# Samirez/Visual_odometry

Hardware: AMD Instinct MI355X
Metric: frame-pairs/sec (1280x720, 2000 ORB feats) (higher is better)
Workload: dtype u8+f32+f64; 1 GPU; seeded synthetic 1280x720 drone flight (256 distinct rendered views, closed loop), 2000 ORB features/frame, 8 levels = BASELINE config 2; chunk of 257 consecutive frames -> 256 pairs (k, k+1) per GPU per step, each frame detected once; detector=orb, distinct_rendered_frames=256, pair_stride=1, contexts_per_gpu=3, keypoint_order=cv2, poly_solver=fast, matcher=crosscheck, matcher_kernel=mfma_fp4, ransac=5-point, conf 0.99, 1 px, seed 2^64-1, <=1000 iters, parallelism=single GPU, pairs_ok_last_step=256

## Files before the change

### visual_odometry_amd/csrc/orb_kernels.hip

```cpp
#include "vo_internal.h"
#include <type_traits>
#include <float.h>
#include <stdlib.h>

__constant__ int8_t c_pattern[256 * 4] = {
#include "orb_pattern.inc"
};
__constant__ int c_umax[16] = {15, 15, 15, 15, 14, 14, 14, 13, 13, 12, 11, 10, 9, 8, 6, 3};
__constant__ int c_gauss7[7] = {18, 34, 49, 55, 49, 34, 18};


typedef short vo_s16x2 __attribute__((ext_vector_type(2)));
typedef unsigned short vo_u16x2 __attribute__((ext_vector_type(2)));
__device__ __forceinline__ uint32_t pk_sub16(uint32_t a, uint32_t b)
{
    return __builtin_bit_cast(uint32_t, __builtin_bit_cast(vo_s16x2, a) - __builtin_bit_cast(vo_s16x2, b));
}
__device__ __forceinline__ uint32_t pk_add16(uint32_t a, uint32_t b)
{
    return __builtin_bit_cast(uint32_t, __builtin_bit_cast(vo_s16x2, a) + __builtin_bit_cast(vo_s16x2, b));
}
__device__ __forceinline__ uint32_t pk_min16(uint32_t a, uint32_t b)
{
    return __builtin_bit_cast(uint32_t, __builtin_elementwise_min(__builtin_bit_cast(vo_s16x2, a), __builtin_bit_cast(vo_s16x2, b)));
}
__device__ __forceinline__ uint32_t pk_max16(uint32_t a, uint32_t b)
{
    return __builtin_bit_cast(uint32_t, __builtin_elementwise_max(__builtin_bit_cast(vo_s16x2, a), __builtin_bit_cast(vo_s16x2, b)));
}
__device__ __forceinline__ uint32_t pk_lshr16_8(uint32_t a)
{
    return __builtin_bit_cast(uint32_t, __builtin_bit_cast(vo_u16x2, a) >> (unsigned short)8);
}
__device__ __forceinline__ uint32_t swap16(uint32_t a) { return __builtin_amdgcn_alignbit(a, a, 16); }

__device__ __forceinline__ int wave_incl_scan(int v, int lane)
{
#pragma unroll
    for (int d = 1; d < 64; d <<= 1) {
        int t = __shfl_up(v, d, 64);
        if (lane >= d) v += t;
    }
    return v;
}

__device__ __forceinline__ int block_excl_scan(int v, int* s_w, int* total)
{
    const int tid = threadIdx.x, lane = tid & 63, wid = tid >> 6, nw = (blockDim.x + 63) >> 6;
    int inc = wave_incl_scan(v, lane);
    __syncthreads();
    if (lane == 63) s_w[wid] = inc;
    __syncthreads();
    if (wid == 0) {
        int w = lane < nw ? s_w[lane] : 0;
        int winc = wave_incl_scan(w, lane);
        if (lane < nw) s_w[lane] = winc - w;
        if (lane == nw - 1) s_w[16] = winc;
    }
// ... 1045 lines not shown
    const LevelGeom lv = g.lv[l];
    const int n = min(ff.cand_count[f * VO_MAX_LEVELS + l], lv.cand_cap);
    const uint32_t* pos = ff.cand_pos + (size_t)f * g.cand_total + lv.cand_off;
    const float* resp = ff.cand_resp + (size_t)f * g.cand_total + lv.cand_off;
    const float thr = thr_in[f * VO_MAX_LEVELS + l];
    int out_base = 0;
    for (int k = 0; k < l; k++) out_base += kept_in[f * VO_MAX_LEVELS + k];
    uint32_t* kp_pos = ff.kp_pos + (size_t)f * g.kp_cap;
    int* kp_level = ff.kp_level + (size_t)f * g.kp_cap;
    float* kp_resp = ff.kp_resp + (size_t)f * g.kp_cap;
    bool overflow = false;
    for (int base = 0; base < n; base += 256) {
        const int i = base + tid;
        const bool keep = i < n && resp[i] >= thr;
        int tot;
        const int p = out_base + block_excl_scan(keep ? 1 : 0, s_w, &tot);
        if (keep) {
            if (p < g.kp_cap) { kp_pos[p] = pos[i]; kp_level[p] = l; kp_resp[p] = resp[i]; }
            else overflow = true;
        }
        out_base += tot;
    }
    if (overflow) atomicOr(&ff.flags[f], 1);
    if (l == g.nlevels - 1 && tid == 0) ff.kp_count[f] = min(out_base, g.kp_cap);
}

void launch_select_harris(hipStream_t s, const PyrGeom& g, FrameFeat ff, int F, float* thr, int* kept)
{
    hipLaunchKernelGGL(k_harris_threshold, dim3(g.nlevels, F), dim3(256), 0, s, g, ff, thr, kept);
    hipLaunchKernelGGL(k_harris_compact, dim3(g.nlevels, F), dim3(256), 0, s, g, ff, thr, kept);
}

__device__ __forceinline__ float fast_atan2_deg(float y, float x)
{
    const float p1 = 0.9997878412794807f * (float)(180 / 3.1415926535897932384626433832795);
    const float p3 = -0.3258083974640975f * (float)(180 / 3.1415926535897932384626433832795);
    const float p5 = 0.1555786518463281f * (float)(180 / 3.1415926535897932384626433832795);
    const float p7 = -0.04432655554792128f * (float)(180 / 3.1415926535897932384626433832795);
    float ax = fabsf(x), ay = fabsf(y), a, c, c2;
    if (ax >= ay) {
        c = ay / (ax + (float)DBL_EPSILON);
        c2 = c * c;
        a = (((p7 * c2 + p5) * c2 + p3) * c2 + p1) * c;
    } else {
        c = ax / (ay + (float)DBL_EPSILON);
        c2 = c * c;
        a = 90.f - (((p7 * c2 + p5) * c2 + p3) * c2 + p1) * c;
    }
    if (x < 0) a = 180.f - a;
    if (y < 0) a = 360.f - a;
    return a;
}

__constant__ uint32_t c_disc_mask[16][8] = {
#define DM(u0, um) ((((u0) >= -(um) && (u0) <= (um)) ? 0x000000ffu : 0u) | (((u0) + 1 >= -(um) && (u0) + 1 <= (um)) ? 0x0000ff00u : 0u) | \
                    (((u0) + 2 >= -(um) && (u0) + 2 <= (um)) ? 0x00ff0000u : 0u) | (((u0) + 3 >= -(um) && (u0) + 3 <= (um)) ? 0xff000000u : 0u))
#define DROW(um) {DM(-15, um), DM(-11, um), DM(-7, um), DM(-3, um), DM(1, um), DM(5, um), DM(9, um), DM(13, um)}
    DROW(15), DROW(15), DROW(15), DROW(15), DROW(14), DROW(14), DROW(14), DROW(13),
    DROW(13), DROW(12), DROW(11), DROW(10), DROW(9), DROW(8), DROW(6), DROW(3)
#undef DROW
#undef DM
};

#ifndef ANG_KPW
#define ANG_KPW 4
#endif
__global__ __launch_bounds__(256) void k_angle(const uint8_t* pyr, PyrGeom g, FrameFeat ff, int blocks_per_frame)
{
    const int bid = xcd_tile(blockIdx.x, gridDim.x);
    const int f = bid / blocks_per_frame, lane = threadIdx.x & 63;
    const int k0 = ((bid % blocks_per_frame) * 4 + (threadIdx.x >> 6)) * ANG_KPW;
    const int cnt = min(ff.kp_count[f], g.kp_cap);
    if (k0 >= cnt) return;
    const uint8_t* corner[ANG_KPW];
    int stride[ANG_KPW];
#pragma unroll
    for (int q = 0; q < ANG_KPW; q++) {
        const size_t ki = (size_t)f * g.kp_cap + min(k0 + q, cnt - 1);
        const uint32_t pos = __builtin_amdgcn_readfirstlane(ff.kp_pos[ki]);
        const int level = __builtin_amdgcn_readfirstlane(ff.kp_level[ki]);
        stride[q] = g.lv[level].stride;
        corner[q] = pyr + (size_t)f * g.frame_bytes + g.lv[level].off + (size_t)((int)(pos >> 16) - 15) * stride[q] + ((int)(pos & 0xffff) - 15);
    }
    uint32_t w[ANG_KPW][4];
#pragma unroll
    for (int q = 0; q < ANG_KPW; q++)
#pragma unroll
        for (int it = 0; it < 4; it++) {
            const int idx = min(it * 64 + lane, 247);
            __builtin_memcpy(&w[q][it], corner[q] + (size_t)(idx >> 3) * stride[q] + 4 * (idx & 7), 4);
        }
    float m10f = 0.f, m01f = 0.f;
#pragma unroll
    for (int q = 0; q < ANG_KPW; q++) {
        int m10 = 0, m01 = 0;
#pragma unroll
        for (int it = 0; it < 4; it++) {
            const int idx = it * 64 + lane;
            const int r = min(idx, 247) >> 3, j = idx & 7, v = r - 15, av = v < 0 ? -v : v;
            const uint32_t x = idx < 248 ? w[q][it] & c_disc_mask[av][j] : 0u;
            const int sum = (int)__builtin_amdgcn_udot4(x, 0x01010101u, 0u, false);
            const int wsum = (int)__builtin_amdgcn_udot4(x, 0x03020100u, 0u, false);
            m10 += (4 * j - 15) * sum + wsum;
            m01 += v * sum;
        }
#pragma unroll
        for (int d = 32; d >= 1; d >>= 1) { m10 += __shfl_xor(m10, d, 64); m01 += __shfl_xor(m01, d, 64); }
        if (lane == q) { m10f = (float)m10; m01f = (float)m01; }
    }
    if (lane < ANG_KPW && k0 + lane < cnt) ff.kp_angle[(size_t)f * g.kp_cap + k0 + lane] = fast_atan2_deg(m01f, m10f);
}

void launch_angle(hipStream_t s, const uint8_t* pyr, const PyrGeom& g, FrameFeat ff, int F)
{
    const int bpf = (g.kp_cap + 4 * ANG_KPW - 1) / (4 * ANG_KPW);
    hipLaunchKernelGGL(k_angle, dim3(bpf * F), dim3(256), 0, s, pyr, g, ff, bpf);
}

__device__ __forceinline__ int reflect101(int i, int n)
{
    if (n == 1) return 0;
    while (i < 0 || i >= n) i = i < 0 ? -i : 2 * n - 2 - i;
    return i;
}

#define BL_INW 160
#define BL_INH (BLUR_TH + 6)
#define BL_ROWS_PER_LANE (BLUR_TH / 8)

__global__ __launch_bounds__(256) void k_blur(const uint8_t* pyr, uint8_t* blur, PyrGeom g)
{
    __shared__ __attribute__((aligned(16))) uint8_t s_in[BL_INH * BL_INW];
    __shared__ __attribute__((aligned(16))) uint16_t s_h[BL_INH * BLUR_TW];
    const int f = blockIdx.y, tid = threadIdx.x;
    const int bid = xcd_tile(blockIdx.x, g.btiles_total);
    int l = 0;
    while (l + 1 < g.nlevels && bid >= g.lv[l + 1].btile_base) l++;
    const LevelGeom lv = g.lv[l];
    const int tile = bid - lv.btile_base;
    const int x0 = (tile % lv.btiles_x) * BLUR_TW, y0 = (tile / lv.btiles_x) * BLUR_TH;
    const uint8_t* img = pyr + (size_t)f * g.frame_bytes + lv.off;
    if (lv.w >= 16 && lv.h >= 4) {
        {
            constexpr int NCH = BL_INW / 16, RPS = 256 / NCH, NLD = (BL_INH + RPS - 1) / RPS;
            const int cc = tid % NCH, rr = tid / NCH;
            const bool lane_ok = tid < RPS * NCH;
            const int gx = x0 - 16 + 16 * cc;
            const bool inx = gx >= 0 && gx + 16 <= lv.stride;
            const uint8_t* src = img + min(max(gx, 0), lv.stride - 16);
            const bool rows_inside = y0 >= 3 && y0 + BLUR_TH + 3 <= lv.h;
            uint4 bv[NLD];
#pragma unroll
            for (int k = 0; k < NLD; k++) {
                const int ry = min(rr + RPS * k, BL_INH - 1);
                const int gy = rows_inside ? y0 - 3 + ry : reflect101(y0 - 3 + ry, lv.h);
                const uint4 v = *(const uint4*)(src + (size_t)gy * lv.stride);
                bv[k] = inx ? v : make_uint4(0, 0, 0, 0);
            }
#pragma unroll
            for (int k = 0; k < NLD; k++)
                if (lane_ok && rr + RPS * k < BL_INH) *(uint4*)(s_in + (rr + RPS * k) * BL_INW + 16 * cc) = bv[k];
        }
        const bool left = x0 == 0, right = x0 + BLUR_TW + 3 > lv.w;
        if (left || right) {
            __syncthreads();
            for (int i = tid; i < BL_INH * 6; i += 256) {
                const int ry = i / 6, k = i % 6;
                if (k < 3) {
                    if (left) s_in[ry * BL_INW + 16 - 3 + k] = s_in[ry * BL_INW + 16 + 3 - k];
                } else if (right) {
                    const int x = lv.w + (k - 3), sx = 2 * lv.w - 2 - x;
// ... 174 lines not shown
    const LevelGeom lv = g.lv[l];
    const int ntx = (lv.stride + 255) / 256, tile = wt - first;
    const int x0 = (tile % ntx) * 256, y0 = (tile / ntx) * BD_R;
    const int x = x0 + 4 * lane;
    const uint8_t* img = pyr + (size_t)f * g.frame_bytes + lv.off;
    const int xb = min(max(x - 4, 0), lv.stride - 12);
    BdEdge e;
    e.left = x0 == 0; e.right = x0 + 256 + 8 > lv.w;
    e.shl = x == 0; e.shr = x - 4 > lv.stride - 12 && x < lv.stride;
    {
        const int d = lv.w - x;
        e.s1 = d == 1 ? 0x01020304u : d == 2 ? 0x03040504u : d == 3 ? 0x05060504u : 0x07060504u;
        e.s2 = d == 2 ? 0x0c0c0c02u : d == 3 ? 0x0c0c0304u : 0x0c040506u;
        e.s3 = d == 5 ? 0x01020304u : d == 6 ? 0x03040504u : 0x07060504u;
        e.use_t = d >= 2 && d <= 4;
    }
    const __amdgpu_buffer_rsrc_t drs = __builtin_amdgcn_make_buffer_rsrc(blur + (size_t)f * g.frame_bytes + lv.off, 0, lv.stride * lv.h, 0x00020000);
    const bool col_ok = x < lv.stride;
    const int nout = min(BD_R, lv.h - y0);
    const int nsteps = (nout + 1) / 2;
    const bool inside = y0 >= 3 && y0 - 3 + 2 * (nsteps + 3 + BD_AHEAD) <= lv.h, edge = e.left || e.right;
    if (inside && !edge) bd_strip<true, false>(img, lv, drs, x, xb, y0, nout, nsteps, col_ok, e);
    else if (inside) bd_strip<true, true>(img, lv, drs, x, xb, y0, nout, nsteps, col_ok, e);
    else if (!edge) bd_strip<false, false>(img, lv, drs, x, xb, y0, nout, nsteps, col_ok, e);
    else bd_strip<false, true>(img, lv, drs, x, xb, y0, nout, nsteps, col_ok, e);
}

void launch_blur(hipStream_t s, const uint8_t* pyr, uint8_t* blur, const PyrGeom& g, int F)
{
    bool direct = true;
    int total = 0;
    for (int l = 0; l < g.nlevels; l++) {
        direct = direct && g.lv[l].w >= 16 && g.lv[l].h >= 8;
        total += ((g.lv[l].stride + 255) / 256) * ((g.lv[l].h + BD_R - 1) / BD_R);
    }
    if (direct) { hipLaunchKernelGGL(k_blur_direct, dim3((total + 3) / 4, F), dim3(256), 0, s, pyr, blur, g, total); return; }
    hipLaunchKernelGGL(k_blur, dim3(g.btiles_total, F), dim3(256), 0, s, pyr, blur, g);
}

__device__ __forceinline__ uint32_t brief_expand4(uint32_t nib)
{
    const uint32_t m = (nib * 0x00204081u) & 0x01010101u;
    return 0x81818181u ^ (m * 0xfeu);
}

__device__ __forceinline__ uint32_t brief_expand8_fp4(uint32_t b)
{
    uint32_t w = (b | (b << 12)) & 0x000F000Fu;
    w = (w | (w << 6)) & 0x03030303u;
    w = (w | (w << 3)) & 0x11111111u;
    return 0xAAAAAAAAu ^ (w << 3);
}

__global__ __launch_bounds__(256) void k_brief_trig(PyrGeom g, FrameFeat ff)
{
    const int f = blockIdx.y, k = blockIdx.x * 256 + threadIdx.x;
    if (k >= min(ff.kp_count[f], g.kp_cap)) return;
    const size_t ki = (size_t)f * g.kp_cap + k;
    const float angle = ff.kp_angle[ki] * (float)(3.1415926535897932384626433832795 / 180.f);
    ff.kp_xy[ki * 2] = (float)cos((double)angle);
    ff.kp_xy[ki * 2 + 1] = (float)sin((double)angle);
}

#define BR_R 18
#define BR_ROWS (2 * BR_R + 1)
#ifndef BR_KPW
#define BR_KPW 2
#endif
__global__ __launch_bounds__(256) void k_brief(const uint8_t* blur, PyrGeom g, FrameFeat ff, uint8_t* desc_x, int cap_x, int blocks_per_frame, int fp4)
{
    __shared__ __attribute__((aligned(16))) uint8_t s_win[4][BR_KPW][BR_ROWS * 64];
    const int bid = xcd_tile(blockIdx.x, gridDim.x);
    const int f = bid / blocks_per_frame, lane = threadIdx.x & 63, wave = threadIdx.x >> 6;
    const int k0 = ((bid % blocks_per_frame) * 4 + wave) * BR_KPW;
    const int cnt = min(ff.kp_count[f], g.kp_cap);
    if (k0 >= cnt) return;
    float ca[BR_KPW], cb[BR_KPW], kxs[BR_KPW], kys[BR_KPW], sfs[BR_KPW];
    int coff[BR_KPW];
    uint4 wv[BR_KPW][3];
#pragma unroll
    for (int q = 0; q < BR_KPW; q++) {
        const size_t ki = (size_t)f * g.kp_cap + min(k0 + q, cnt - 1);
        const uint32_t pos = __builtin_amdgcn_readfirstlane(ff.kp_pos[ki]);
        const int level = __builtin_amdgcn_readfirstlane(ff.kp_level[ki]);
        const float sf = g.lv[level].scale;
        const int stride = g.lv[level].stride, lh = g.lv[level].h;
        const float kx = (float)(pos & 0xffff) * sf, ky = (float)(pos >> 16) * sf;
        const float inv = 1.f / sf;
        const int cx = __float2int_rn(kx * inv), cy = __float2int_rn(ky * inv);
        ca[q] = ff.kp_xy[ki * 2]; cb[q] = ff.kp_xy[ki * 2 + 1];
        kxs[q] = kx; kys[q] = ky; sfs[q] = sf;
        const uint8_t* img = blur + (size_t)f * g.frame_bytes + g.lv[level].off;
        const int xs = (cx - BR_R) & ~15;
        const int nchunk = (cx - BR_R - xs) + 2 * BR_R + 1 > 48 ? 4 : 3;
        coff[q] = BR_R * 64 + (cx - xs);
#pragma unroll
        for (int it = 0; it < 3; it++) {
            const int idx = min(it * 64 + lane, BR_ROWS * 4 - 1);
            const int r = idx >> 2, c = idx & 3;
            const int gy = min(max(cy - BR_R + r, 0), lh - 1), gx = min(max(xs + (c < nchunk ? 16 * c : 0), 0), stride - 16);
            wv[q][it] = *(const uint4*)(img + (size_t)gy * stride + gx);
        }
    }
#pragma unroll
    for (int q = 0; q < BR_KPW; q++)
#pragma unroll
        for (int it = 0; it < 3; it++) {
            const int idx = it * 64 + lane;
            if (idx < BR_ROWS * 4) *(uint4*)(s_win[wave][q] + idx * 16) = wv[q][it];
        }
#pragma unroll
    for (int q = 0; q < BR_KPW; q++) {
        const int k = k0 + q;
        if (k >= cnt) break;
        const size_t ki = (size_t)f * g.kp_cap + k;
        const uint8_t* center = s_win[wave][q] + coff[q];
        const float a = ca[q], b = cb[q];
        uint64_t words[4];
#pragma unroll
        for (int w = 0; w < 4; w++) {
            const int8_t* pt = c_pattern + (w * 64 + lane) * 4;
            const float px0 = (float)pt[0], py0 = (float)pt[1], px1 = (float)pt[2], py1 = (float)pt[3];
            const float xa = px0 * a - py0 * b, ya = px0 * b + py0 * a;
            const float xb = px1 * a - py1 * b, yb = px1 * b + py1 * a;
            const int t0 = center[__float2int_rn(ya) * 64 + __float2int_rn(xa)];
            const int t1 = center[__float2int_rn(yb) * 64 + __float2int_rn(xb)];
            words[w] = __ballot(t0 < t1);
        }
        if (lane < 4) {
            uint64_t wv8 = lane == 0 ? words[0] : lane == 1 ? words[1] : lane == 2 ? words[2] : words[3];
            *(uint64_t*)(ff.desc + ki * 32 + lane * 8) = wv8;
        }
        if (fp4 < 0) {
        } else if (fp4) {
            if (lane < 8) {
                const uint64_t wv8 = lane < 2 ? words[0] : lane < 4 ? words[1] : lane < 6 ? words[2] : words[3];
                const uint32_t bits = (uint32_t)(wv8 >> (32 * (lane & 1)));
                const uint4 o = make_uint4(brief_expand8_fp4(bits & 255u), brief_expand8_fp4((bits >> 8) & 255u), brief_expand8_fp4((bits >> 16) & 255u), brief_expand8_fp4(bits >> 24));
                *(uint4*)(desc_x + ((size_t)f * cap_x * 16 + (size_t)(k & ~15) * 8 + (size_t)lane * 16 + (k & 15)) * 16) = o;
            }
        } else if (lane < 16) {
            const uint64_t wv8 = lane < 4 ? words[0] : lane < 8 ? words[1] : lane < 12 ? words[2] : words[3];
            const uint32_t bits = (uint32_t)(wv8 >> (16 * (lane & 3))) & 0xffffu;
            const uint4 o = make_uint4(brief_expand4(bits & 15u), brief_expand4((bits >> 4) & 15u), brief_expand4((bits >> 8) & 15u), brief_expand4(bits >> 12));
            *(uint4*)(desc_x + (((size_t)f * cap_x + (k & ~15)) * 16 + (size_t)lane * 16 + (k & 15)) * 16) = o;
        }
        if (lane == 0) {
            ff.kp_xy[ki * 2] = kxs[q]; ff.kp_xy[ki * 2 + 1] = kys[q];
            ff.kp_size[ki] = 31 * sfs[q];
        }
    }
}

void launch_brief(hipStream_t s, const uint8_t* blur, const PyrGeom& g, FrameFeat ff, int F, uint8_t* desc_x, int cap_x, int fp4)
{
    hipLaunchKernelGGL(k_brief_trig, dim3((g.kp_cap + 255) / 256, F), dim3(256), 0, s, g, ff);
    const int bpf = (g.kp_cap + 4 * BR_KPW - 1) / (4 * BR_KPW);
    hipLaunchKernelGGL(k_brief, dim3(bpf * F), dim3(256), 0, s, blur, g, ff, desc_x, cap_x, bpf, -1);
    launch_desc_expand(s, ff.desc, ff.kp_count, g.kp_cap, cap_x, desc_x, F, fp4);
}
```

### visual_odometry_amd/csrc/vo_api.hip

```cpp
#include "vo_host.h"

static const char* k_stage_names[VO_STAGE_COUNT] = {
    "gray", "pyramid_resize", "fast_score_nms", "select_fast", "harris", "select_harris", "ic_angle",
    "gaussian_blur", "rbrief", "match_nn", "match_select", "essential_ransac", "recover_pose",
    "triangulate", "misc", "reserved", "sift_scale_space", "sift_extrema", "sift_refine_orient", "sift_sort_unique",
    "sift_descriptor", "cv2_keypoint_order", "trajectory_gather", "reserved2", "slam_ba_prepare", "slam_bundle_adjust", "slam_filter",
    "slam_camera_limit", "slam_map_statistics", "undistort_points"};

static void clear_last_run(vo_ctx* ctx) { ctx->last = LastRun(); }

static void slam_stream_slots_written(vo_ctx* ctx, int first, int n)
{
    for (int k = first < 0 ? 0 : first; k < first + n && k < (int)ctx->undistorted.size(); k++) ctx->undistorted[(size_t)k] = 0;
    SlamStream& st = ctx->stream_map;
    if (st.live && st.anchor >= first && st.anchor < first + n) st.touched = true;
    for (SlamStream::Seq& q : st.seq)
        if (st.live && q.anchor >= first && q.anchor < first + n) q.touched = true;
}

void prof_collect(vo_ctx* c)
{
    for (int i = 0; i < c->n_ev; i++) {
        float ms = 0;
        if (hipEventElapsedTime(&ms, c->ev[i][0], c->ev[i][1]) == hipSuccess) {
// ... 449 lines not shown
    HIPCHK(hipStreamSynchronize(ctx->stream));
    if (ctx->prof) prof_collect(ctx);
    return VO_OK;
}

static int run_detect(vo_ctx* ctx, int first_slot, int F, int upto)
{
    const PyrGeom& g = ctx->g;
    hipStream_t s = ctx->stream;
    uint8_t* pyr = ctx->pyr + (size_t)first_slot * g.frame_bytes;
    uint8_t* blur = ctx->blur + (size_t)first_slot * g.frame_bytes;
    uint8_t* score = ctx->score + (size_t)first_slot * g.frame_bytes;
    FrameFeat ff = ctx->ff;
    ff.cand_pos += (size_t)first_slot * g.cand_total; ff.cand_resp += (size_t)first_slot * g.cand_total;
    ff.cand_count += (size_t)first_slot * VO_MAX_LEVELS;
    ff.kp_pos += (size_t)first_slot * g.kp_cap; ff.kp_level += (size_t)first_slot * g.kp_cap;
    ff.kp_resp += (size_t)first_slot * g.kp_cap; ff.kp_angle += (size_t)first_slot * g.kp_cap;
    ff.kp_xy += (size_t)first_slot * g.kp_cap * 2; ff.kp_size += (size_t)first_slot * g.kp_cap;
    ff.desc += (size_t)first_slot * g.kp_cap * 32;
    ff.kp_count += first_slot; ff.flags += first_slot;
    ff.hist += (size_t)first_slot * VO_MAX_LEVELS * 256;
    ff.tile_list += (size_t)first_slot * g.ftiles_total * FAST_LISTCAP; ff.tile_count += (size_t)first_slot * g.ftiles_total;
    {
        StageTimer t(ctx, ST_RESIZE);
        for (int l = 1; l < g.nlevels; l++) launch_resize(s, pyr, g, l, ctx->tabs[l], F);
    }
    if (upto < 1) return VO_OK;
    const bool cv2 = ctx->kp_order == 1 && ctx->cv2_ready;
    Cv2Buf cb = ctx->cv2;
    if (cv2) {
        const size_t fo = (size_t)first_slot;
        cb.all_pos += fo * cb.all_total; cb.all_resp += fo * cb.all_total; cb.work += fo * cb.all_total;
        cb.all_cand += fo * cb.all_total; cb.lpos += fo * cb.all_total; cb.rpos += fo * cb.all_total;
        cb.all_count += fo * VO_MAX_LEVELS; cb.chunk_count += fo * g.sel_chunks_total;
    }
    {
        StageTimer t(ctx, ST_MISC);
        HIPCHK(hipMemsetAsync(ff.hist, 0, (size_t)F * VO_MAX_LEVELS * 256 * sizeof(uint32_t), s));
        if (upto < 2) {
            HIPCHK(hipMemsetAsync(ff.flags, 0, (size_t)F * sizeof(int), s));
            HIPCHK(hipMemsetAsync(ff.cand_count, 0, (size_t)F * VO_MAX_LEVELS * sizeof(int), s));
            if (cv2) HIPCHK(hipMemsetAsync(cb.all_count, 0, (size_t)F * VO_MAX_LEVELS * sizeof(int), s));
        }
    }
    { StageTimer t(ctx, ST_FAST); launch_fast(s, pyr, score, ff.hist, g, F, upto < 2 ? nullptr : ff.tile_list, ff.tile_count); }
    if (upto < 2) return VO_OK;
    { StageTimer t(ctx, ST_SELECT_FAST); launch_select_fast(s, g, ff, F, ctx->sel_thr + (size_t)first_slot * VO_MAX_LEVELS, ctx->sel_chunk_count + (size_t)first_slot * g.sel_chunks_total, ff.tile_list, ff.tile_count, cv2 ? &cb : nullptr); }
    if (g.score_type == 0) { StageTimer t(ctx, ST_HARRIS); launch_harris(s, pyr, g, ff, F); }
    { StageTimer t(ctx, ST_SELECT_HARRIS); launch_select_harris(s, g, ff, F, ctx->har_thr + (size_t)first_slot * VO_MAX_LEVELS, ctx->har_kept + (size_t)first_slot * VO_MAX_LEVELS); }
    if (cv2) {
        StageTimer t(ctx, ST_CV2_ORDER);
        launch_cv2_order(s, g, ff, cb, F, ctx->har_kept + (size_t)first_slot * VO_MAX_LEVELS);
    }
    { StageTimer t(ctx, ST_ANGLE); launch_angle(s, pyr, g, ff, F); }
    { StageTimer t(ctx, ST_BLUR); launch_blur(s, pyr, blur, g, F); }
    {
        StageTimer t(ctx, ST_BRIEF);
        const int cx = desc_x_rows(g.kp_cap);
        const int fp4 = descx_begin_write(ctx, first_slot, F);
        launch_brief(s, blur, g, ff, F, ctx->desc_x + (size_t)first_slot * cx * 256, cx, fp4);
    }
    return VO_OK;
}

extern "C" int vo_batch_kp_capacity(vo_ctx* ctx)
{
    if (!ctx) return 0;
    const Batch b = batch(ctx);
    return b.ready ? b.kp_cap : 0;
}

extern "C" int vo_host_alloc(size_t bytes, void** out)
{
    if (!out) return VO_ERR_INVALID;
    *out = nullptr;
    return hipHostMalloc(out, bytes ? bytes : 1, hipHostMallocDefault) == hipSuccess ? VO_OK : VO_ERR_HIP;
}

extern "C" void vo_host_free(void* p)
{
    if (p) (void)hipHostFree(p);
}

static int detect_enqueue(vo_ctx* ctx, int first_slot, int F)
{
    const Batch b = batch(ctx);
    if (!b.ready) FAIL(VO_ERR_NOT_CONFIGURED, "vo_batch_configure has not been called");
    if (F < 0 || first_slot < 0 || first_slot + F > b.max_frames) FAIL(VO_ERR_INVALID, "slot range out of bounds");
    slam_stream_slots_written(ctx, first_slot, F);
    HIPCHK(hipSetDevice(ctx->device));
    if (F == 0) return VO_OK;
    if (b.sift) return sift_frames_detect_enqueue(ctx, first_slot, F);
    int rc = run_detect(ctx, first_slot, F, 2);
    if (rc) return rc;
    HIPCHK(hipGetLastError());
    return VO_OK;
}

extern "C" int vo_frames_detect_async(vo_ctx* ctx, int first_slot, int F)
{
    if (!ctx) return VO_ERR_INVALID;
    int rc = detect_enqueue(ctx, first_slot, F);
    if (rc) return rc;
    HIPCHK(hipEventRecord(ctx->ev_det, ctx->stream));
    ctx->ev_det_set = true;
    return VO_OK;
}

extern "C" int vo_detect_after(vo_ctx* ctx, vo_ctx* other)
{
    if (!ctx || !other) return VO_ERR_INVALID;
    if (ctx->device != other->device) FAIL(VO_ERR_INVALID, "the two contexts are on different devices");
    if (ctx == other || !other->ev_det_set) return VO_OK;
// ... 2019 lines not shown
    ctx->n_ev = 0;
    return VO_OK;
}

extern "C" int vo_profile_reset(vo_ctx* ctx)
{
    if (!ctx) return VO_ERR_INVALID;
    memset(ctx->prof_ms, 0, sizeof(ctx->prof_ms));
    memset(ctx->prof_n, 0, sizeof(ctx->prof_n));
    ctx->n_ev = 0;
    return VO_OK;
}

extern "C" int vo_profile_read(vo_ctx* ctx, float* ms, int32_t* launches)
{
    if (!ctx || !ms || !launches) return VO_ERR_INVALID;
    memcpy(ms, ctx->prof_ms, sizeof(ctx->prof_ms));
    memcpy(launches, ctx->prof_n, sizeof(ctx->prof_n));
    return VO_OK;
}

extern "C" const char* vo_stage_name(int stage)
{
    return stage >= 0 && stage < VO_STAGE_COUNT ? k_stage_names[stage] : "?";
}

extern "C" double vo_stage_bytes(vo_ctx* ctx, int stage, int F)
{
    const Batch bt = ctx ? batch(ctx) : Batch{};
    if (bt.sift && bt.ready) {
        const SiftState& S = ctx->sift;
        const int L = S.P.nLayers;
        double px = 0;
        for (int o = 0; o < S.P.nOct; o++) px += (double)S.P.w[o] * S.P.h[o];
        const double p0 = (double)S.P.w[0] * S.P.h[0];
        double b = 0;
        if (stage == ST_SIFT_SCALE) b = (double)S.w * S.h + 4.0 * p0 * 3 + 4.0 * px * ((L + 2) + (L + 2)) + 4.0 * (px - p0) * 1.25;
        else if (stage == ST_SIFT_EXTREMA) b = 4.0 * px * (L + 3);
        else if (stage == ST_MATCH_NN) b = 2.0 * S.kp_cap * 128;
        else if (stage == ST_UNDISTORT) b = 16.0 * S.kp_cap;
        return b * F;
    }
    if (!ctx || !ctx->configured) return 0.0;
    const PyrGeom& g = ctx->g;
    double px[VO_MAX_LEVELS], total = 0;
    for (int l = 0; l < g.nlevels; l++) { px[l] = (double)g.lv[l].w * g.lv[l].h; total += px[l]; }
    const double N = g.nfeatures;
    double b = 0;
    switch (stage) {
    case ST_RESIZE: b = (total - px[g.nlevels - 1]) + (total - px[0]); break;
    case ST_FAST: b = total; break;
    case ST_SELECT_FAST: b = 2 * 2 * N * 12; break;
    case ST_HARRIS: b = 2 * N * 81 + 2 * N * 4; break;
    case ST_ANGLE: b = N * 749; break;
    case ST_BLUR: b = total + total; break;
    case ST_BRIEF: b = N * 512 + N * 32 + N * 28; break;
    case ST_MATCH_NN: b = 2 * N * 32; break;
    case ST_MATCH_SELECT: b = 16 * N; break;
    case ST_RANSAC: b = 33 * N; break;
    case ST_POSE: b = 32 * N; break;
    case ST_UNDISTORT: b = 16 * N; break;
    default: b = 0;
    }
    return b * F;
}
```

### visual_odometry_amd/csrc/vo_internal.h

```cpp
#pragma once
#include <hip/hip_runtime.h>
#include <stdint.h>
#include "../../include/vo_hip.h"

enum {
    ST_GRAY = 0, ST_RESIZE, ST_FAST, ST_SELECT_FAST, ST_HARRIS, ST_SELECT_HARRIS, ST_ANGLE,
    ST_BLUR, ST_BRIEF, ST_MATCH_NN, ST_MATCH_SELECT, ST_RANSAC, ST_POSE, ST_TRIANGULATE,
    ST_MISC, ST_RESERVED, ST_SIFT_SCALE, ST_SIFT_EXTREMA, ST_SIFT_ORIENT, ST_SIFT_SORT, ST_SIFT_DESC, ST_CV2_ORDER, ST_GATHER, ST_RESERVED2,
    ST_SLAM_PREPARE, ST_SLAM_BA, ST_SLAM_FILTER, ST_SLAM_LIMIT, ST_SLAM_STATS, ST_UNDISTORT
};

struct LevelGeom {
    int w, h, stride, off;
    int quota;
    float scale;
    int ftile_base, ftiles_x;
    int fox, foy;
    int dtile_base, dtiles_x;
    int btile_base, btiles_x;
    int cand_off, cand_cap;
    int sel_chunk_base;
};

struct PyrGeom {
// ... 77 lines not shown
    int*      nn_dist2;
    int*      nn_colkey;
    int*      m_q;
    int*      m_t;
    float*    m_d;
    int*      m_count;
    double*   px1;
    double*   px2;
    double*   xn1;
    double*   xn2;
    uint8_t*  mask;
    double*   models;
    PoseState* pose_state;
    double*   in1;
    double*   in2;
    double*   ipx1;
    double*   ipx2;
    vo_pair_result* res;
    double*   X;
    uint8_t*  pose_mask;
};

struct RansacParams {
    double prob, thresh_px;
    int max_iters;
    uint64_t seed;
    double K[9];
    double dist_thresh;
    int dk_early;
};

const char* rccl_load(void);
const char* rccl_unique_id(uint8_t* id128);
const char* rccl_comm_init(void** comm, const uint8_t* id128, int rank, int world);
void rccl_comm_destroy(void* comm);
const char* rccl_comm_count(void* comm, int* n);
const char* rccl_all_gather_f64(void* comm, const double* send, double* recv, size_t count, hipStream_t s);
void launch_pack_records(hipStream_t s, const vo_pair_result* res, int B, int valid, double* rec);

void launch_gray(hipStream_t s, const uint8_t* src, int channels, int row_stride, int64_t frame_stride,
                 uint8_t* pyr, const PyrGeom& g, int F);
void launch_gray_plain(hipStream_t s, const uint8_t* src, int channels, int row_stride, int64_t frame_stride,
                       uint8_t* dst, int w, int h, int dstride, int64_t dframe, int F);
void launch_resize(hipStream_t s, uint8_t* pyr, const PyrGeom& g, int level, const ResizeTab& tab, int F);
void launch_fast(hipStream_t s, const uint8_t* pyr, uint8_t* score, uint32_t* hist, const PyrGeom& g, int F,
                 uint32_t* tile_list, int* tile_count);
void launch_select_fast(hipStream_t s, const PyrGeom& g, FrameFeat ff, int F, int* thr, int* chunk_count,
                        const uint32_t* tile_list, const int* tile_count, const Cv2Buf* cb);
void launch_harris(hipStream_t s, const uint8_t* pyr, const PyrGeom& g, FrameFeat ff, int F);
void launch_cv2_order(hipStream_t s, const PyrGeom& g, FrameFeat ff, Cv2Buf cb, int F, const int* kept);
void launch_retain_raw(hipStream_t s, const float* resp, int n, int n_points, uint2* a, uint32_t* lpos, uint32_t* rpos,
                       int* order, int* n_out);
void launch_select_harris(hipStream_t s, const PyrGeom& g, FrameFeat ff, int F, float* thr, int* kept);
void launch_angle(hipStream_t s, const uint8_t* pyr, const PyrGeom& g, FrameFeat ff, int F);
void launch_resize_linear(hipStream_t st, const uint8_t* src, int sw, int sh, int cn, int sstride, int64_t sframe,
                          uint8_t* dst, int dw, int dh, int dstride, int64_t dframe,
                          const int* xofs, const void* xa, const int* yofs, const void* yb, int area2, int F);
void launch_resize_area(hipStream_t st, const uint8_t* src, int cn, int sstride, uint8_t* dst, int dw, int dh, int dstride,
                        int isx, int isy, const int* xsi, const float* xal, const int* xst, const int* ysi, const float* yal, const int* yst);
#define SIFT_IMG_BORDER 5
#define SIFT_MAX_INTERP_STEPS 5
#define SIFT_MAX_OCT 16
#define SIFT_MAX_TAPS 64
struct SiftGeom {
    int nOct, nLayers;
    int w[SIFT_MAX_OCT], h[SIFT_MAX_OCT], stride[SIFT_MAX_OCT];
    size_t plane[SIFT_MAX_OCT];
    size_t goff[SIFT_MAX_OCT];
    size_t gframe;
};
struct SiftCand { int o, layer, r, c; };
struct SiftKp { float x, y, size, angle, response; int octave; };
struct SiftSurv { SiftKp kp; int o, layer, r, c; };
struct SiftExpTab { float tab[64]; };
int launch_sb_sweep_base(hipStream_t s, const uint8_t* img, int channels, int row_stride, int64_t frame_stride, int sw, int sh,
                         float* dstG, size_t g_fs, int stride, int F, const float* taps, int ntaps);
int launch_sb_sweep(hipStream_t s, const float* src, size_t src_fs, float* dstG, size_t g_fs, int w, int h, int stride, int F,
                    const float* taps, int ntaps, float* dstH = nullptr, size_t h_fs = 0, int hstride = 0, int hw = 0, int hh = 0);
void launch_sb_extrema(hipStream_t s, const SiftGeom& P, const float* gauss, int o, float threshold, SiftCand* cand, int* counts, int cap, int F);
void launch_sb_refine_orient(hipStream_t s, const SiftGeom& P, const float* gauss, const SiftCand* cand, int cand_cap, float contrastThr,
                             float edgeThr, float sigma, const SiftExpTab& E, SiftSurv* surv, int surv_cap, SiftKp* kps, int kp_cap, int* counts, int F, int waves);
void launch_sb_sort_emit(hipStream_t s, const SiftKp* kps, int kp_cap, int* counts, int* rank , void* rank_tmp , SiftKp* sorted,
                         SiftKp* out, int out_cap, int* out_count, int* out_flags, int cand_cap, int surv_cap, int F);
void launch_sb_descriptor(hipStream_t s, const SiftGeom& P, const float* gauss, const SiftKp* kps, int kp_cap, const int* counts, const SiftExpTab& E,
                          uint8_t* desc, uint8_t* desc_x, int cap_x, int* norms, int* flags, int first_slot, int F, int waves);
void launch_sb_pack_rows(hipStream_t s, const uint8_t* rows, int n, int slot, int kp_cap, uint8_t* desc, uint8_t* desc_x, int cap_x, int* norms, int* flags);
void launch_sb_unpack(hipStream_t s, const SiftKp* kps, int kp_cap, const int* counts, int first_slot, float* kp_xy, float* kp_size, float* kp_angle,
                      float* kp_resp, int* kp_oct, int* kp_count, const int* fin_count, const int* fin_flags, int* flags, int F);
void launch_match_nn_l2i8(hipStream_t s, const uint8_t* desc_x, const int* norms, const int* kp_count, int kp_cap, int cap_x, PairBuf pb, int P,
                          int dirs_mask, int knn2);

#include "jpeg_host.h"
void launch_jpeg_decode(hipStream_t s, const uint8_t* blob, JpegImage* imgs, const JpegTables* tabs, int F, uint8_t* clean, uint32_t* rst,
                        int16_t* coef, uint8_t* planes, uint8_t* out, int max_blocks, int max_w, int max_h, bool gray = false,
                        bool packed_tables = false ,
                        hipEvent_t coef_cleared = nullptr );

void launch_pnp_ransac(hipStream_t s, const double* obj, const double* img, const int* offsets, int B, const double* Kd,
                       int iterations, double reproj_err, double confidence, uint64_t seed, const uint32_t* rng_tab, int rng_n,
                       int refine_cv2, double* rvec, double* tvec, uint8_t* mask, int* ninl, int* status, int off_stride = 1);
void launch_rodrigues(hipStream_t s, const double* in, int in_is_matrix, double* out);
void launch_blur(hipStream_t s, const uint8_t* pyr, uint8_t* blur, const PyrGeom& g, int F);
void launch_brief(hipStream_t s, const uint8_t* blur, const PyrGeom& g, FrameFeat ff, int F, uint8_t* desc_x, int cap_x, int fp4);

__device__ __forceinline__ int xcd_tile(int b, int n)
{
    const int q = n >> 3, r = n & 7, x = b & 7, k = b >> 3;
    return (x < r ? x * (q + 1) : r * (q + 1) + (x - r) * q) + k;
}

static inline int desc_x_rows(int kp_cap) { return (kp_cap + 255) & ~255; }
void launch_desc_expand(hipStream_t s, const uint8_t* desc, const int* kp_count, int kp_cap, int cap_x, uint8_t* desc_x, int F, int fp4);
int launch_match_nn(hipStream_t s, const uint8_t* desc_x, const int* kp_count, int kp_cap, int cap_x, PairBuf pb, int P,
                    int dirs_mask, int knn2, int fp4);
size_t nn_colkey_ints(int P, int kp_cap);
void launch_match_nn_popcount(hipStream_t s, const uint8_t* desc, const int* kp_count, int kp_cap, PairBuf pb, int P,
                              int dirs_mask, int knn2);
void launch_match_select(hipStream_t s, const float* kp_xy, const int* kp_count, int kp_cap, PairBuf pb, int P,
                         int mode, double ratio, const double* K, int l2 = 0,
                         int col_parts = 0);

size_t nn_l2_knn2_keys(int na, int nb);
void launch_nn_l2_knn2(hipStream_t s, const float* A, int na, const float* B, int nb, int dim, int* idx, float* dist, unsigned long long* part);
void launch_nn_l2(hipStream_t s, const float* A, int na, const float* B, int nb, int dim, int* idx, float* dist, unsigned long long* key);

void launch_ransac(hipStream_t s, PairBuf pb, int kp_cap, int P, RansacParams rp, const uint32_t* rng_tab, int rng_n);
void launch_pose(hipStream_t s, PairBuf pb, int kp_cap, int P, RansacParams rp);
void launch_triangulate_pairs(hipStream_t s, PairBuf pb, int kp_cap, int P, RansacParams rp);
void launch_triangulate_raw(hipStream_t s, const double* P1, const double* P2, const double* x1, const double* x2,
                            int M, double* X);
void launch_five_point_raw(hipStream_t s, const double* x1, const double* x2, double* E, int* nm, int dk_early);
void launch_epilines(hipStream_t s, const void* pts, int point_type, int N, const double* F, void* lines);
struct UndistortParams {
    double fx, fy, cx, cy;
    double k1, k2, p1, p2, k3, k4, k5, k6;
    double RR[9];
};
void launch_undistort_points(hipStream_t s, const void* pts, int point_type, int N, UndistortParams up, void* out);
void launch_undistort_frames(hipStream_t s, float* kp_xy, const int* kp_count, int kp_cap, int F, UndistortParams up);
void launch_pairs_epipolar(hipStream_t s, PairBuf pb, int kp_cap, int P, const double* Kd, double* dist, int* n, double* mean, double* sd, double* mx);
void launch_reprojection(hipStream_t s, const double* poses, int ncam, const double* points, int npt, const int* obs_cam,
                         const int* obs_pt, const double* obs_xy, int nobs, const double* Kd, double threshold,
                         double* sqerr, uint8_t* keep, int* bad);
enum { SEG_INIT = 0,
       SEG_FIRST = 1,
       SEG_COUNT = 2,
       SEG_CAUSE = 3 };
struct RestartBuf {
    int*    st;
    int*    segment; int* cause;
    double* seg_poses;
    double* seg_poses_last;
};
struct ChainBuf {
    unsigned long long* parent;
    uint8_t* in_map;
// ... 194 lines not shown
```

Baseline: 105,000 frame-pairs/s.

## Fuse ORB orientation and trig into the BRIEF kernel

Removes the separate k_angle and k_brief_trig kernels and computes the intensity-centroid moments inside k_brief. Each wave loads raw pyramid rows with 16-byte loads, reduces the moments with permlane/DPP, and computes atan2 plus cos/sin once per keypoint through shared memory. Pattern bytes are now held in registers. The goal is to cut two kernel launches and the round trips of angle and trig values through global memory, in exchange for more registers and extra barriers inside the BRIEF kernel.

```diff
diff --git a/visual_odometry_amd/csrc/orb_kernels.hip b/visual_odometry_amd/csrc/orb_kernels.hip
--- a/visual_odometry_amd/csrc/orb_kernels.hip
+++ b/visual_odometry_amd/csrc/orb_kernels.hip
@@ -3,7 +3,7 @@
 #include <float.h>
 #include <stdlib.h>
 
-__constant__ int8_t c_pattern[256 * 4] = {
+__constant__ __attribute__((aligned(16))) int8_t c_pattern[256 * 4] = {
 #include "orb_pattern.inc"
 };
 __constant__ int c_umax[16] = {15, 15, 15, 15, 14, 14, 14, 13, 13, 12, 11, 10, 9, 8, 6, 3};
@@ -1155,71 +1155,6 @@
     return a;
 }
 
-__constant__ uint32_t c_disc_mask[16][8] = {
-#define DM(u0, um) ((((u0) >= -(um) && (u0) <= (um)) ? 0x000000ffu : 0u) | (((u0) + 1 >= -(um) && (u0) + 1 <= (um)) ? 0x0000ff00u : 0u) | \
-                    (((u0) + 2 >= -(um) && (u0) + 2 <= (um)) ? 0x00ff0000u : 0u) | (((u0) + 3 >= -(um) && (u0) + 3 <= (um)) ? 0xff000000u : 0u))
-#define DROW(um) {DM(-15, um), DM(-11, um), DM(-7, um), DM(-3, um), DM(1, um), DM(5, um), DM(9, um), DM(13, um)}
-    DROW(15), DROW(15), DROW(15), DROW(15), DROW(14), DROW(14), DROW(14), DROW(13),
-    DROW(13), DROW(12), DROW(11), DROW(10), DROW(9), DROW(8), DROW(6), DROW(3)
-#undef DROW
-#undef DM
-};
-
-#ifndef ANG_KPW
-#define ANG_KPW 4
-#endif
-__global__ __launch_bounds__(256) void k_angle(const uint8_t* pyr, PyrGeom g, FrameFeat ff, int blocks_per_frame)
-{
-    const int bid = xcd_tile(blockIdx.x, gridDim.x);
-    const int f = bid / blocks_per_frame, lane = threadIdx.x & 63;
-    const int k0 = ((bid % blocks_per_frame) * 4 + (threadIdx.x >> 6)) * ANG_KPW;
-    const int cnt = min(ff.kp_count[f], g.kp_cap);
-    if (k0 >= cnt) return;
-    const uint8_t* corner[ANG_KPW];
-    int stride[ANG_KPW];
-#pragma unroll
-    for (int q = 0; q < ANG_KPW; q++) {
-        const size_t ki = (size_t)f * g.kp_cap + min(k0 + q, cnt - 1);
-        const uint32_t pos = __builtin_amdgcn_readfirstlane(ff.kp_pos[ki]);
-        const int level = __builtin_amdgcn_readfirstlane(ff.kp_level[ki]);
-        stride[q] = g.lv[level].stride;
-        corner[q] = pyr + (size_t)f * g.frame_bytes + g.lv[level].off + (size_t)((int)(pos >> 16) - 15) * stride[q] + ((int)(pos & 0xffff) - 15);
-    }
-    uint32_t w[ANG_KPW][4];
-#pragma unroll
-    for (int q = 0; q < ANG_KPW; q++)
-#pragma unroll
-        for (int it = 0; it < 4; it++) {
-            const int idx = min(it * 64 + lane, 247);
-            __builtin_memcpy(&w[q][it], corner[q] + (size_t)(idx >> 3) * stride[q] + 4 * (idx & 7), 4);
-        }
-    float m10f = 0.f, m01f = 0.f;
-#pragma unroll
-    for (int q = 0; q < ANG_KPW; q++) {
-        int m10 = 0, m01 = 0;
-#pragma unroll
-        for (int it = 0; it < 4; it++) {
-            const int idx = it * 64 + lane;
-            const int r = min(idx, 247) >> 3, j = idx & 7, v = r - 15, av = v < 0 ? -v : v;
-            const uint32_t x = idx < 248 ? w[q][it] & c_disc_mask[av][j] : 0u;
-            const int sum = (int)__builtin_amdgcn_udot4(x, 0x01010101u, 0u, false);
-            const int wsum = (int)__builtin_amdgcn_udot4(x, 0x03020100u, 0u, false);
-            m10 += (4 * j - 15) * sum + wsum;
-            m01 += v * sum;
-        }
-#pragma unroll
-        for (int d = 32; d >= 1; d >>= 1) { m10 += __shfl_xor(m10, d, 64); m01 += __shfl_xor(m01, d, 64); }
-        if (lane == q) { m10f = (float)m10; m01f = (float)m01; }
-    }
-    if (lane < ANG_KPW && k0 + lane < cnt) ff.kp_angle[(size_t)f * g.kp_cap + k0 + lane] = fast_atan2_deg(m01f, m10f);
-}
-
-void launch_angle(hipStream_t s, const uint8_t* pyr, const PyrGeom& g, FrameFeat ff, int F)
-{
-    const int bpf = (g.kp_cap + 4 * ANG_KPW - 1) / (4 * ANG_KPW);
-    hipLaunchKernelGGL(k_angle, dim3(bpf * F), dim3(256), 0, s, pyr, g, ff, bpf);
-}
-
 __device__ __forceinline__ int reflect101(int i, int n)
 {
     if (n == 1) return 0;
@@ -1500,75 +1435,160 @@
     return 0xAAAAAAAAu ^ (w << 3);
 }
 
-__global__ __launch_bounds__(256) void k_brief_trig(PyrGeom g, FrameFeat ff)
-{
-    const int f = blockIdx.y, k = blockIdx.x * 256 + threadIdx.x;
-    if (k >= min(ff.kp_count[f], g.kp_cap)) return;
-    const size_t ki = (size_t)f * g.kp_cap + k;
-    const float angle = ff.kp_angle[ki] * (float)(3.1415926535897932384626433832795 / 180.f);
-    ff.kp_xy[ki * 2] = (float)cos((double)angle);
-    ff.kp_xy[ki * 2 + 1] = (float)sin((double)angle);
-}
-
 #define BR_R 18
 #define BR_ROWS (2 * BR_R + 1)
 #ifndef BR_KPW
 #define BR_KPW 2
 #endif
-__global__ __launch_bounds__(256) void k_brief(const uint8_t* blur, PyrGeom g, FrameFeat ff, uint8_t* desc_x, int cap_x, int blocks_per_frame, int fp4)
-{
-    __shared__ __attribute__((aligned(16))) uint8_t s_win[4][BR_KPW][BR_ROWS * 64];
+#ifndef BR_WAVES
+#define BR_WAVES 4
+#endif
+#define BR_WG (BR_WAVES * BR_KPW)
+typedef uint32_t br_u32x4 __attribute__((ext_vector_type(4)));
+#define BR_RAW_CHUNKS (31 * 3)
+static_assert(BR_KPW >= 1 && BR_WG <= 64, "one lane of the first wavefront per keypoint of the workgroup");
+
+__device__ __forceinline__ int br_reduce4(int a, int b, int c, int d)
+{
+    const auto h = __builtin_amdgcn_permlane32_swap(a, b, false, false);
+    const auto k = __builtin_amdgcn_permlane32_swap(c, d, false, false);
+    const int ab = (int)h[0] + (int)h[1], cd = (int)k[0] + (int)k[1];
+    const auto q = __builtin_amdgcn_permlane16_swap(ab, cd, false, false);
+    int s = (int)q[0] + (int)q[1];
+    s += __builtin_amdgcn_update_dpp(0, s, 0x128, 0xf, 0xf, false);
+    s += __builtin_amdgcn_update_dpp(0, s, 0x124, 0xf, 0xf, false);
+    s += __builtin_amdgcn_update_dpp(0, s, 0x122, 0xf, 0xf, false);
+    s += __builtin_amdgcn_update_dpp(0, s, 0x121, 0xf, 0xf, false);
+    return s;
+}
+
+__device__ __forceinline__ int br_win_chunk(int it, int lane)
+{
+    const int idx = it * 64 + lane;
+    return idx < BR_ROWS * 4 ? idx : idx - (3 * 64 - BR_ROWS * 4);
+}
+
+__global__ __launch_bounds__(64 * BR_WAVES) void k_brief(const uint8_t* pyr, const uint8_t* blur, PyrGeom g, FrameFeat ff, uint8_t* desc_x, int cap_x, int blocks_per_frame, int fp4)
+{
+    __shared__ __attribute__((aligned(16))) uint8_t s_win[BR_WAVES][BR_KPW][BR_ROWS * 64];
+    __shared__ int s_mom[BR_WG][2];
+    __shared__ float s_trig[BR_WG][2];
     const int bid = xcd_tile(blockIdx.x, gridDim.x);
-    const int f = bid / blocks_per_frame, lane = threadIdx.x & 63, wave = threadIdx.x >> 6;
-    const int k0 = ((bid % blocks_per_frame) * 4 + wave) * BR_KPW;
+    const int f = bid / blocks_per_frame, lane = threadIdx.x & 63;
+    const int wave = __builtin_amdgcn_readfirstlane(threadIdx.x >> 6);
+    const int kbase = (bid % blocks_per_frame) * BR_WG, k0 = kbase + wave * BR_KPW;
     const int cnt = min(ff.kp_count[f], g.kp_cap);
-    if (k0 >= cnt) return;
-    float ca[BR_KPW], cb[BR_KPW], kxs[BR_KPW], kys[BR_KPW], sfs[BR_KPW];
-    int coff[BR_KPW];
-    uint4 wv[BR_KPW][3];
+    if (kbase >= cnt) return;
+    int rrow[2], rcol[2], rlo[2], rhi[2];
+#pragma unroll
+    for (int it = 0; it < 2; it++) {
+        const int idx = it * 64 + lane, i2 = min(idx, BR_RAW_CHUNKS - 1);
+        const int r = i2 / 3, c = i2 - 3 * r, av = r < 15 ? 15 - r : r - 15;
+        const int um = (int)((0x3689abcddeeeffffull >> (4 * av)) & 15);
+        rrow[it] = r; rcol[it] = c;
+        rlo[it] = 15 - um - 16 * c;
+        rhi[it] = idx < BR_RAW_CHUNKS ? 15 + um - 16 * c : -64;
+    }
+    uint32_t pat[4];
+#pragma unroll
+    for (int w = 0; w < 4; w++) pat[w] = ((const uint32_t*)c_pattern)[w * 64 + lane];
+    float kxs[BR_KPW], kys[BR_KPW], sfs[BR_KPW];
+    int coff[BR_KPW], roff[BR_KPW], rxs[BR_KPW], ry0[BR_KPW], wxs[BR_KPW], wy0[BR_KPW], nchunk[BR_KPW], stride[BR_KPW], lh[BR_KPW];
+    size_t lvoff[BR_KPW];
 #pragma unroll
     for (int q = 0; q < BR_KPW; q++) {
         const size_t ki = (size_t)f * g.kp_cap + min(k0 + q, cnt - 1);
-        const uint32_t pos = __builtin_amdgcn_readfirstlane(ff.kp_pos[ki]);
-        const int level = __builtin_amdgcn_readfirstlane(ff.kp_level[ki]);
+        const uint32_t pos = ff.kp_pos[ki];
+        const int level = ff.kp_level[ki];
         const float sf = g.lv[level].scale;
-        const int stride = g.lv[level].stride, lh = g.lv[level].h;
-        const float kx = (float)(pos & 0xffff) * sf, ky = (float)(pos >> 16) * sf;
-        const float inv = 1.f / sf;
-        const int cx = __float2int_rn(kx * inv), cy = __float2int_rn(ky * inv);
-        ca[q] = ff.kp_xy[ki * 2]; cb[q] = ff.kp_xy[ki * 2 + 1];
-        kxs[q] = kx; kys[q] = ky; sfs[q] = sf;
-        const uint8_t* img = blur + (size_t)f * g.frame_bytes + g.lv[level].off;
-        const int xs = (cx - BR_R) & ~15;
-        const int nchunk = (cx - BR_R - xs) + 2 * BR_R + 1 > 48 ? 4 : 3;
-        coff[q] = BR_R * 64 + (cx - xs);
+        stride[q] = g.lv[level].stride; lh[q] = g.lv[level].h;
+        lvoff[q] = (size_t)f * g.frame_bytes + g.lv[level].off;
+        const int px = (int)(pos & 0xffff), py = (int)(pos >> 16);
+        kxs[q] = (float)px * sf; kys[q] = (float)py * sf; sfs[q] = sf;
+        rxs[q] = max((px - 15) & ~15, 0); roff[q] = (px - 15) & 15; ry0[q] = max(py - 15, 0);
+        const int xs = max((px - BR_R) & ~15, 0);
+        wxs[q] = xs; wy0[q] = max(py - BR_R, 0);
+        nchunk[q] = (px - BR_R - xs) + 2 * BR_R + 1 > 48 ? 4 : 3;
+        coff[q] = BR_R * 64 + (px - xs);
+    }
+    br_u32x4 rv[BR_KPW][2], wv[BR_KPW][3];
+#pragma unroll
+    for (int q = 0; q < BR_KPW; q++)
+#pragma unroll
+        for (int it = 0; it < 2; it++) {
+            const int gy = min(ry0[q] + rrow[it], lh[q] - 1), gx = min(rxs[q] + 16 * rcol[it], stride[q] - 16);
+            rv[q][it] = *(const br_u32x4*)(pyr + lvoff[q] + (uint32_t)(__mul24(gy, stride[q]) + gx));
+        }
+#pragma unroll
+    for (int q = 0; q < BR_KPW; q++)
 #pragma unroll
         for (int it = 0; it < 3; it++) {
-            const int idx = min(it * 64 + lane, BR_ROWS * 4 - 1);
+            const int idx = br_win_chunk(it, lane);
             const int r = idx >> 2, c = idx & 3;
-            const int gy = min(max(cy - BR_R + r, 0), lh - 1), gx = min(max(xs + (c < nchunk ? 16 * c : 0), 0), stride - 16);
-            wv[q][it] = *(const uint4*)(img + (size_t)gy * stride + gx);
-        }
+            const int gy = min(wy0[q] + r, lh[q] - 1), gx = min(wxs[q] + (c < nchunk[q] ? 16 * c : 0), stride[q] - 16);
+            wv[q][it] = *(const br_u32x4*)(blur + lvoff[q] + (uint32_t)(__mul24(gy, stride[q]) + gx));
+        }
+    int m10[BR_KPW], m01[BR_KPW];
+#pragma unroll
+    for (int q = 0; q < BR_KPW; q++) {
+        m10[q] = 0; m01[q] = 0;
+#pragma unroll
+        for (int it = 0; it < 2; it++) {
+            const int lo = max(roff[q] + rlo[it], 0), hi = min(roff[q] + rhi[it], 15);
+            const uint32_t bm = hi >= 0 ? ((2u << hi) - 1u) & (0xffffffffu << lo) : 0u;
+            const uint32_t x4[4] = {rv[q][it].x, rv[q][it].y, rv[q][it].z, rv[q][it].w};
+            uint32_t sum = 0u, wsum = 0u;
+#pragma unroll
+            for (int d = 0; d < 4; d++) {
+                const uint32_t t = __umul24((bm >> (4 * d)) & 15u, 0x00204081u) & 0x01010101u;
+                const uint32_t x = x4[d] & ((0x80808080u - t) ^ 0x80808080u);
+                sum = __builtin_amdgcn_udot4(x, 0x01010101u, sum, false);
+                wsum = __builtin_amdgcn_udot4(x, 0x03020100u + 0x04040404u * d, wsum, false);
+            }
+            m10[q] += __mul24(16 * rcol[it] - roff[q] - 15, (int)sum) + (int)wsum;
+            m01[q] += __mul24(rrow[it] - 15, (int)sum);
+        }
+    }
+#pragma unroll
+    for (int q = 0; q < BR_KPW; q += 2) {
+        const bool two = q + 1 < BR_KPW;
+        const int s = br_reduce4(m10[q], m01[q], two ? m10[q + 1] : 0, two ? m01[q + 1] : 0);
+        const int row = lane >> 4;
+        if ((lane & 15) == 0 && (two || !(row & 1))) s_mom[wave * BR_KPW + q + (row & 1)][row >> 1] = s;
     }
 #pragma unroll
     for (int q = 0; q < BR_KPW; q++)
 #pragma unroll
         for (int it = 0; it < 3; it++) {
-            const int idx = it * 64 + lane;
-            if (idx < BR_ROWS * 4) *(uint4*)(s_win[wave][q] + idx * 16) = wv[q][it];
-        }
+            *(br_u32x4*)(s_win[wave][q] + br_win_chunk(it, lane) * 16) = wv[q][it];
+        }
+    float ptx0[4], pty0[4], ptx1[4], pty1[4];
+#pragma unroll
+    for (int w = 0; w < 4; w++) {
+        ptx0[w] = (float)(int8_t)(pat[w] & 0xff); pty0[w] = (float)(int8_t)((pat[w] >> 8) & 0xff);
+        ptx1[w] = (float)(int8_t)((pat[w] >> 16) & 0xff); pty1[w] = (float)(int8_t)(pat[w] >> 24);
+    }
+    __syncthreads();
+    if (threadIdx.x < BR_WG) {
+        const int k = kbase + (int)threadIdx.x;
+        const float angle = fast_atan2_deg((float)s_mom[threadIdx.x][1], (float)s_mom[threadIdx.x][0]);
+        if (k < cnt) ff.kp_angle[(size_t)f * g.kp_cap + k] = angle;
+        const float a = angle * (float)(3.1415926535897932384626433832795 / 180.f);
+        s_trig[threadIdx.x][0] = (float)cos((double)a);
+        s_trig[threadIdx.x][1] = (float)sin((double)a);
+    }
+    __syncthreads();
 #pragma unroll
     for (int q = 0; q < BR_KPW; q++) {
         const int k = k0 + q;
         if (k >= cnt) break;
         const size_t ki = (size_t)f * g.kp_cap + k;
         const uint8_t* center = s_win[wave][q] + coff[q];
-        const float a = ca[q], b = cb[q];
+        const float a = s_trig[wave * BR_KPW + q][0], b = s_trig[wave * BR_KPW + q][1];
         uint64_t words[4];
 #pragma unroll
         for (int w = 0; w < 4; w++) {
-            const int8_t* pt = c_pattern + (w * 64 + lane) * 4;
-            const float px0 = (float)pt[0], py0 = (float)pt[1], px1 = (float)pt[2], py1 = (float)pt[3];
+            const float px0 = ptx0[w], py0 = pty0[w], px1 = ptx1[w], py1 = pty1[w];
             const float xa = px0 * a - py0 * b, ya = px0 * b + py0 * a;
             const float xb = px1 * a - py1 * b, yb = px1 * b + py1 * a;
             const int t0 = center[__float2int_rn(ya) * 64 + __float2int_rn(xa)];
@@ -1600,10 +1620,9 @@
     }
 }
 
-void launch_brief(hipStream_t s, const uint8_t* blur, const PyrGeom& g, FrameFeat ff, int F, uint8_t* desc_x, int cap_x, int fp4)
-{
-    hipLaunchKernelGGL(k_brief_trig, dim3((g.kp_cap + 255) / 256, F), dim3(256), 0, s, g, ff);
-    const int bpf = (g.kp_cap + 4 * BR_KPW - 1) / (4 * BR_KPW);
-    hipLaunchKernelGGL(k_brief, dim3(bpf * F), dim3(256), 0, s, blur, g, ff, desc_x, cap_x, bpf, -1);
+void launch_brief(hipStream_t s, const uint8_t* pyr, const uint8_t* blur, const PyrGeom& g, FrameFeat ff, int F, uint8_t* desc_x, int cap_x, int fp4)
+{
+    const int bpf = (g.kp_cap + BR_WG - 1) / BR_WG;
+    hipLaunchKernelGGL(k_brief, dim3(bpf * F), dim3(64 * BR_WAVES), 0, s, pyr, blur, g, ff, desc_x, cap_x, bpf, -1);
     launch_desc_expand(s, ff.desc, ff.kp_count, g.kp_cap, cap_x, desc_x, F, fp4);
 }
diff --git a/visual_odometry_amd/csrc/vo_api.hip b/visual_odometry_amd/csrc/vo_api.hip
--- a/visual_odometry_amd/csrc/vo_api.hip
+++ b/visual_odometry_amd/csrc/vo_api.hip
@@ -525,13 +525,12 @@
         StageTimer t(ctx, ST_CV2_ORDER);
         launch_cv2_order(s, g, ff, cb, F, ctx->har_kept + (size_t)first_slot * VO_MAX_LEVELS);
     }
-    { StageTimer t(ctx, ST_ANGLE); launch_angle(s, pyr, g, ff, F); }
     { StageTimer t(ctx, ST_BLUR); launch_blur(s, pyr, blur, g, F); }
     {
         StageTimer t(ctx, ST_BRIEF);
         const int cx = desc_x_rows(g.kp_cap);
         const int fp4 = descx_begin_write(ctx, first_slot, F);
-        launch_brief(s, blur, g, ff, F, ctx->desc_x + (size_t)first_slot * cx * 256, cx, fp4);
+        launch_brief(s, pyr, blur, g, ff, F, ctx->desc_x + (size_t)first_slot * cx * 256, cx, fp4);
     }
     return VO_OK;
 }
@@ -2657,9 +2656,8 @@
     case ST_FAST: b = total; break;
     case ST_SELECT_FAST: b = 2 * 2 * N * 12; break;
     case ST_HARRIS: b = 2 * N * 81 + 2 * N * 4; break;
-    case ST_ANGLE: b = N * 749; break;
     case ST_BLUR: b = total + total; break;
-    case ST_BRIEF: b = N * 512 + N * 32 + N * 28; break;
+    case ST_BRIEF: b = N * 749 + N * 512 + N * 32 + N * 28; break;
     case ST_MATCH_NN: b = 2 * N * 32; break;
     case ST_MATCH_SELECT: b = 16 * N; break;
     case ST_RANSAC: b = 33 * N; break;
diff --git a/visual_odometry_amd/csrc/vo_internal.h b/visual_odometry_amd/csrc/vo_internal.h
--- a/visual_odometry_amd/csrc/vo_internal.h
+++ b/visual_odometry_amd/csrc/vo_internal.h
@@ -153,7 +153,6 @@
 void launch_retain_raw(hipStream_t s, const float* resp, int n, int n_points, uint2* a, uint32_t* lpos, uint32_t* rpos,
                        int* order, int* n_out);
 void launch_select_harris(hipStream_t s, const PyrGeom& g, FrameFeat ff, int F, float* thr, int* kept);
-void launch_angle(hipStream_t s, const uint8_t* pyr, const PyrGeom& g, FrameFeat ff, int F);
 void launch_resize_linear(hipStream_t st, const uint8_t* src, int sw, int sh, int cn, int sstride, int64_t sframe,
                           uint8_t* dst, int dw, int dh, int dstride, int64_t dframe,
                           const int* xofs, const void* xa, const int* yofs, const void* yb, int area2, int F);
@@ -202,7 +201,7 @@
                        int refine_cv2, double* rvec, double* tvec, uint8_t* mask, int* ninl, int* status, int off_stride = 1);
 void launch_rodrigues(hipStream_t s, const double* in, int in_is_matrix, double* out);
 void launch_blur(hipStream_t s, const uint8_t* pyr, uint8_t* blur, const PyrGeom& g, int F);
-void launch_brief(hipStream_t s, const uint8_t* blur, const PyrGeom& g, FrameFeat ff, int F, uint8_t* desc_x, int cap_x, int fp4);
+void launch_brief(hipStream_t s, const uint8_t* pyr, const uint8_t* blur, const PyrGeom& g, FrameFeat ff, int F, uint8_t* desc_x, int cap_x, int fp4);
 
 __device__ __forceinline__ int xcd_tile(int b, int n)
 {
```

Measured after the change: 108,000 frame-pairs/s, median of 6. 1.03x the previous value.
